# muellan/metacache

Measured on AMD Instinct MI355X. Metric: Mreads/min (150 bp), higher is better.
Workload: dtype u32

## Files before the change

### metacache_amd/csrc/gw_kernels.hip

```cpp
#include "device_common.h"

#include <algorithm>
#include <cstdlib>

namespace mcamd {

namespace {

constexpr uint32_t kGwNone = 0xFFFFFFFFu;
constexpr uint32_t kGwRounds = 128;
constexpr uint32_t kGwLoads = kGwRounds / 16;

struct __attribute__((packed, aligned(4))) U4 { uint32_t x, y, z, w; };

__device__ __forceinline__ uint32_t gw_block_shift(uint32_t maxWin)
{
    const uint32_t D = maxWin > 1 ? maxWin - 1 : 1;
    const uint32_t A = 32u - (uint32_t)__builtin_clz(64u * D - 1u);
    return A < 8u ? 8u : A;
}

template <uint32_t T1LOG2, uint32_t T2LOG2>
struct GwBloom {
    static constexpr uint32_t kW1 = (1u << T1LOG2) / 32, kW2 = (1u << T2LOG2) / 32, kWords = kW1 + kW2;
// ... 572 lines not shown
__device__ __forceinline__ uint32_t gw_count_numbers(const uint32_t (&v)[PER], uint2* slots, uint32_t* ck, const uint32_t lane)
{
    constexpr uint32_t kByteMask = ((1u << LOG2S) - 1u) << 3;
    char* base = reinterpret_cast<char*>(slots);
    auto key_at = [&](uint32_t off) -> uint32_t* { return reinterpret_cast<uint32_t*>(base + off); };
    uint32_t off[PER], old[PER];
    bool coll = false;
#pragma unroll
    for (uint32_t r = 0; r < PER; ++r) {
        off[r] = gw_slot<LOG2S>(v[r]);
        old[r] = v[r] != kGwNone ? atomicCAS(key_at(off[r]), kGwNone, v[r]) : v[r];
        coll = coll || (old[r] != kGwNone && old[r] != v[r]);
    }
    if (__ballot(coll)) {
#pragma unroll
        for (uint32_t r = 0; r < PER; ++r) {
            if (old[r] != kGwNone && old[r] != v[r]) {
                uint32_t o = off[r];
                for (;;) {
                    o = (o + 8u) & kByteMask;
                    old[r] = atomicCAS(key_at(o), kGwNone, v[r]);
                    if (old[r] == kGwNone || old[r] == v[r]) break;
                }
                off[r] = o;
            }
        }
    }
    uint32_t C = 0;
#pragma unroll
    for (uint32_t r = 0; r < PER; ++r) {
        if (v[r] != kGwNone) atomicAdd(key_at(off[r]) + 1, 1u);
        const bool claimed = v[r] != kGwNone && old[r] == kGwNone;
        const uint64_t m = __ballot(claimed);
        if (claimed) {
            const uint32_t at = __builtin_amdgcn_mbcnt_hi((uint32_t)(m >> 32), __builtin_amdgcn_mbcnt_lo((uint32_t)m, C));
            if (CKCAP == 0xFFFFFFFFu || at < CKCAP) ck[at] = off[r];
        }
        C += (uint32_t)__popcll(m);
    }
    return C;
}

template <uint32_t LOG2S, uint32_t PER, bool TAX>
__device__ __forceinline__ uint32_t gw_pick(const uint32_t* ck, const uint32_t C, uint2* slots, const uint32_t lane, const uint32_t maxWin,
                                            const uint32_t K, const uint32_t* __restrict__ taxkey, const DeviceTable& tab,
                                            uint32_t& owv, uint32_t& owh, uint32_t& owd)
{
    constexpr uint32_t kByteMask = ((1u << LOG2S) - 1u) << 3;
    const char* base = reinterpret_cast<const char*>(slots);
    uint32_t v[PER], R[PER];
#pragma unroll
    for (uint32_t r = 0; r < PER; ++r) {
        const uint2 c = r * 64 + lane < C ? *reinterpret_cast<const uint2*>(base + ck[r * 64 + lane]) : make_uint2(kGwNone, 0u);
        v[r] = c.x; R[r] = c.y;
    }
    uint32_t tgt[TAX ? PER : 1], thi[TAX ? PER : 1];
    if constexpr (TAX) {
#pragma unroll
        for (uint32_t r = 0; r < PER; ++r) tgt[r] = v[r] != kGwNone ? tab.gwDir[v[r] >> tab.gwDirShift] : 0u;
    }
    for (uint32_t d = 1; d < maxWin; ++d) {
        uint2 kc[PER]; uint32_t o[PER];
        bool chain = false;
#pragma unroll
        for (uint32_t r = 0; r < PER; ++r) {
            o[r] = gw_slot<LOG2S>(v[r] - d);
            kc[r] = *reinterpret_cast<const uint2*>(base + o[r]);
            if (v[r] == kGwNone) kc[r].x = kGwNone;
            chain = chain || (kc[r].x != v[r] - d && kc[r].x != kGwNone);
        }
        if (__ballot(chain)) {
#pragma unroll
            for (uint32_t r = 0; r < PER; ++r)
                while (kc[r].x != v[r] - d && kc[r].x != kGwNone) { o[r] = (o[r] + 8u) & kByteMask; kc[r] = *reinterpret_cast<const uint2*>(base + o[r]); }
        }
#pragma unroll
        for (uint32_t r = 0; r < PER; ++r)
            if (kc[r].x == v[r] - d) R[r] = ((R[r] & 0xFFFFu) + kc[r].y) | (d << 16);
    }
    uint32_t ptax[TAX ? PER : 1];
    if constexpr (TAX) {
#pragma unroll
        for (uint32_t r = 0; r < PER; ++r) {
            thi[r] = v[r] != kGwNone ? tab.gwBase[tgt[r] + 1] : 0u;
            while (v[r] != kGwNone && v[r] >= thi[r]) { ++tgt[r]; thi[r] = tab.gwBase[tgt[r] + 1]; }
            ptax[r] = v[r] != kGwNone ? taxkey[tgt[r]] : 0u;
        }
    }
    uint32_t live = 0;
#pragma unroll
    for (uint32_t r = 0; r < PER; ++r) {
        bool ok = v[r] != kGwNone;
        if constexpr (TAX) ok = ok && ptax[r] != 0;
        live |= ok ? (1u << r) : 0u;
    }
    uint32_t strong = 0;
    uint32_t wv = kGwNone, wh = 0, wd = 0;
    for (uint32_t rnd = 0; rnd < K; ++rnd) {
        uint32_t hh = 0, hv = kGwNone, hd = 0, hg = 0;
#pragma unroll
        for (uint32_t r = 0; r < PER; ++r) {
            const uint32_t h = R[r] & 0xFFFFu;
            const bool take = ((live >> r) & 1u) && (h > hh || (h == hh && v[r] < hv));
            if (take) { hh = h; hv = v[r]; hd = R[r] >> 16; if constexpr (TAX) hg = ptax[r]; }
        }
        const uint32_t mh = wave_max_u32(hh);
        if (mh == 0) break;
        const uint32_t mv = wave_min_u32(hh == mh ? hv : kGwNone);
        const uint32_t winner = __ffsll((unsigned long long)__ballot(hh == mh && hv == mv)) - 1;
        const uint32_t d = rdlane(hd, winner);
        if constexpr (TAX) {
            const uint32_t g = rdlane(hg, winner);
#pragma unroll
            for (uint32_t r = 0; r < PER; ++r) if (ptax[r] == g) live &= ~(1u << r);
        } else {
            const uint32_t from = mv - tab.gwGap, span = 2u * tab.gwGap;
#pragma unroll
            for (uint32_t r = 0; r < PER; ++r) if (v[r] - from <= span) live &= ~(1u << r);
        }
        if (lane == rnd) { wv = mv; wh = mh; wd = d; }
        strong += mh >= 2 ? 1u : 0u;
    }
    owv = wv; owh = wh; owd = wd;
    return strong;
}

template <bool TAX>
__device__ __forceinline__ bool gw_winners_out(const uint32_t lane, const uint32_t K, const uint32_t wv, const uint32_t wh, const uint32_t wd,
                                               const uint32_t wt, const uint32_t wlo, const uint32_t whi, mc_candidate_dev* __restrict__ out,
                                               uint32_t (&pickLo)[kLaneK], uint32_t (&pickHi)[kLaneK])
{
    bool again = false;
    if constexpr (!TAX) {
#pragma unroll
        for (uint32_t i = 0; i + 1 < kLaneK; ++i) {
            const uint32_t ti = rdlane(wt, i);
            again = again || (__ballot(lane > i && lane < K && wt == ti && ti != 0xFFFFFFFFu) != 0);
        }
    }
#pragma unroll
    for (uint32_t i = 0; i < kLaneK; ++i) { pickLo[i] = rdlane(wlo, i); pickHi[i] = rdlane(whi, i); }
    if (lane < K) {
        mc_candidate_dev e; e.tgt = wt; e.hits = wh; e.end = wv - wlo; e.beg = e.end - wd;
        if (wv == kGwNone) { e.tgt = 0xFFFFFFFFu; e.hits = 0; e.beg = 0; e.end = 0; }
        out[lane] = e;
    }
    return again;
}

}

namespace {

struct GwPend {
    bool pend = false;
    uint32_t q = 0, wv = kGwNone, wh = 0, wd = 0, dir = 0, b0 = 0, b1 = 0, b2 = 0;
    __device__ __forceinline__ void bases(const DeviceTable& tab)
    {
        if (pend && wv != kGwNone) { b0 = tab.gwBase[dir]; b1 = tab.gwBase[dir + 1]; b2 = tab.gwBase[min(dir + 2, tab.gwTargets)]; }
    }
    template <bool TAX>
    __device__ __forceinline__ void finish(const uint32_t lane, const uint32_t K, const DeviceTable& tab, const Workspace& ws, mc_candidate_dev* __restrict__ cands)
    {
        if (!pend) return;
        uint32_t t = 0xFFFFFFFFu, lo = 0, hi = 0;
        if (wv != kGwNone) {
            t = dir; lo = b0; hi = b1;
            if (wv >= b1) { ++t; lo = b1; hi = b2; }
            while (wv >= hi) { ++t; lo = hi; hi = tab.gwBase[t + 1]; }
        }
        uint32_t plo[kLaneK], phi[kLaneK];
        const bool again = gw_winners_out<TAX>(lane, K, wv, wh, wd, t, lo, hi, cands + (size_t)q * K, plo, phi);
        if (lane == 0) {
            if (again) { ws.hitScan[q] = ws.qstat[q].hits; ws.qflag[q] = kFlagCands; }
            else ws.qflag[q] = kFlagDone;
        }
        pend = false;
    }
};

template <uint32_t LOG2S, bool TAX, bool DEFER, bool LONG = false, class GetV, class EntF>
__device__ __forceinline__ bool gw_count_read(const uint32_t q, EntF&& entf, const uint32_t n2, const uint32_t maxWin, GetV&& getv,
                                              uint2* slots, uint32_t* ck, uint64_t* T, const uint32_t lane, const uint32_t grp, const uint32_t sub4,
                                              const uint32_t K, const uint32_t* __restrict__ taxkey, const DeviceTable& tab, const Workspace& ws,
                                              mc_candidate_dev* __restrict__ cands, GwPend& P)
{
    constexpr uint32_t kSlots = 1u << LOG2S, kList = kSlots / 2;
    {
        uint4* k4 = reinterpret_cast<uint4*>(slots);
#pragma unroll
        for (uint32_t i = 0; i < kSlots * 8 / 16 / 64; ++i) k4[i * 64 + lane] = make_uint4(kGwNone, 0u, kGwNone, 0u);
    }
    wave_lds_sync();
    uint32_t pickLo[kLaneK], pickHi[kLaneK];
#pragma unroll
    for (uint32_t i = 0; i < kLaneK; ++i) { pickLo[i] = 0; pickHi[i] = 0; }
    uint32_t strong = 0, wv = kGwNone, wh = 0, wd = 0;
    bool again = false;
    mc_candidate_dev* out = cands + (size_t)q * K;
    if constexpr (DEFER) P.bases(tab);
    uint32_t C = 0;
    auto body = [&](auto perc) {
        constexpr uint32_t PER = decltype(perc)::value;
        uint32_t v[PER];
#pragma unroll
        for (uint32_t r = 0; r < PER; ++r) v[r] = getv(r);
        C = gw_count_numbers<LOG2S, PER, LONG ? kList : 0xFFFFFFFFu>(v, slots, ck, lane);
    };
    const uint32_t per = (n2 + 63u) / 64u;
    if constexpr (LOG2S == 9) {
        if (per <= 1) body(std::integral_constant<uint32_t, 1>{});
        else if (per <= 2) body(std::integral_constant<uint32_t, 2>{});
        else if (per <= 3) body(std::integral_constant<uint32_t, 3>{});
        else if (!LONG || per <= 4) body(std::integral_constant<uint32_t, 4>{});
        else if constexpr (LONG) {
            if (per <= 6) body(std::integral_constant<uint32_t, 6>{});
            else body(std::integral_constant<uint32_t, 8>{});
        }
    } else if constexpr (LOG2S == 10) {
        if (per <= 6) body(std::integral_constant<uint32_t, 6>{});
        else body(std::integral_constant<uint32_t, 8>{});
    } else {
        if (per <= 10) body(std::integral_constant<uint32_t, 10>{});
        else if (per <= 12) body(std::integral_constant<uint32_t, 12>{});
        else body(std::integral_constant<uint32_t, kList / 64>{});
    }
    C = __builtin_amdgcn_readfirstlane(C);
    wave_lds_sync();
    if constexpr (LONG) {
        if (C > kList) {
            if constexpr (DEFER) P.template finish<TAX>(lane, K, tab, ws, cands);
            wave_lds_sync();
            return false;
        }
    }
    auto pick = [&](auto perc) {
        constexpr uint32_t PER = decltype(perc)::value;
        strong = gw_pick<LOG2S, PER, TAX>(ck, C, slots, lane, maxWin, K, taxkey, tab, wv, wh, wd);
    };
    if (C <= 64) pick(std::integral_constant<uint32_t, 1>{});
    else if (C <= 128) pick(std::integral_constant<uint32_t, 2>{});
    else if (C <= 256) pick(std::integral_constant<uint32_t, 4>{});
    else if constexpr (LOG2S >= 10) {
        if (C <= 512) pick(std::integral_constant<uint32_t, 8>{});
        else if constexpr (LOG2S >= 11) pick(std::integral_constant<uint32_t, 16>{});
    }
    strong = __builtin_amdgcn_readfirstlane(strong);
    if constexpr (DEFER) {
        P.template finish<TAX>(lane, K, tab, ws, cands);
        if (strong >= K) {
            P.pend = true; P.q = q; P.wv = wv; P.wh = wh; P.wd = wd;
            P.dir = wv != kGwNone ? tab.gwDir[wv >> tab.gwDirShift] : 0u;
            wave_lds_sync();
            return true;
        }
    }
    {
        uint32_t wt = 0xFFFFFFFFu, wlo = 0, whi = 0;
        if (wv != kGwNone) tab.gw_target_bounds(wv, wt, wlo, whi);
        again = gw_winners_out<TAX>(lane, K, wv, wh, wd, wt, wlo, whi, out, pickLo, pickHi);
    }
    bool done = true;
    if (again) {
        if (lane == 0) { ws.hitScan[q] = ws.qstat[q].hits; ws.qflag[q] = kFlagCands; }
        done = false;
    } else if (strong < K) {
        const uint2 r6 = entf();
        const uint32_t fbase = r6.x, nent = r6.y;
        if (TAX || nent > kBigEnt) {
            if (lane == 0) { ws.hitScan[q] = ws.qstat[q].hits; ws.qflag[q] = kFlagCands; }
            done = false;
        } else if constexpr (!TAX) {
            wave_lds_sync();
            const uint32_t sz = lane < nent ? (ws.psize[fbase + lane] & 0xFFFFu) : 0u;
            const uint64_t pay = lane < nent ? ws.ppay[fbase + lane] : 0ull;
            const uint32_t myR = sz > 1 ? (sz + 15u) >> 4 : 0u;
            const uint32_t incl = wave_incl_scan_u32(myR, lane), Rc = rdlane(incl, 63), start = incl - myR;
            uint32_t best[kLaneK];
#pragma unroll
            for (uint32_t i = 0; i < kLaneK; ++i) best[i] = kGwNone;
            uint32_t seen = 0;
            auto visit = [&](uint32_t g, bool valid) {
                if (!valid) return;
                bool skip = false;
#pragma unroll
                for (uint32_t i = 0; i < kLaneK; ++i) skip = skip || (i < strong && g - pickLo[i] < pickHi[i] - pickLo[i]);
                if (skip) return;
                ++seen;
                uint32_t c = g;
#pragma unroll
                for (uint32_t i = 0; i < kLaneK; ++i) { const uint32_t lo = min(best[i], c); c = max(best[i], c); best[i] = lo; }
            };
            visit(sz == 1 ? tab.gw_of(pay) : kGwNone, sz == 1);
            for (uint32_t r0 = 0; r0 < Rc; r0 += kGwRounds) {
                for (uint32_t i = lane; i < kGwRounds; i += 64) if (r0 + i >= Rc) T[i] = 0ull;
                const uint32_t jlo = r0 > start ? r0 - start : 0u, jhi = min(myR, r0 + kGwRounds > start ? r0 + kGwRounds - start : 0u);
                for (uint32_t j = jlo; j < jhi; ++j) T[start + j - r0] = (pay + 16ull * j) | ((uint64_t)min(16u, sz - 16u * j) << 40);
                wave_lds_sync();
#pragma unroll
                for (uint32_t u = 0; u < kGwLoads; ++u) {
                    const uint64_t rd = T[u * 16 + grp];
                    const int32_t rem = (int32_t)(uint32_t)(rd >> 40) - (int32_t)sub4;
                    if (rem > 0) {
                        const U4 t = *reinterpret_cast<const U4*>(tab.values32 + (rd & 0xFFFFFFFFFFull) + sub4);
                        visit(t.x, true); visit(t.y, rem > 1); visit(t.z, rem > 2); visit(t.w, rem > 3);
                    }
                }
                wave_lds_sync();
            }
            const bool dropped = seen > kLaneK;
            bool unsure = false;
            for (uint32_t rnd = strong; rnd < K; ++rnd) {
                if (__ballot(dropped && best[0] == kGwNone)) { unsure = true; break; }
                const uint32_t m = wave_min_u32(best[0]);
                mc_candidate_dev e; e.tgt = 0xFFFFFFFFu; e.hits = 0; e.beg = 0; e.end = 0;
                if (m != kGwNone) {
                    const uint32_t t = tab.gw_target(m), lo = tab.gwBase[t], hi = tab.gwBase[t + 1];
                    e.tgt = t; e.hits = 1; e.beg = e.end = m - lo;
                    uint32_t kept[kLaneK];
#pragma unroll
                    for (uint32_t i = 0; i < kLaneK; ++i) kept[i] = kGwNone;
                    uint32_t n = 0;
#pragma unroll
                    for (uint32_t i = 0; i < kLaneK; ++i) {
                        const bool stay = best[i] != kGwNone && !(best[i] - lo < hi - lo);
#pragma unroll
                        for (uint32_t j = 0; j < kLaneK; ++j) if (stay && j == n) kept[j] = best[i];
                        n += stay ? 1u : 0u;
                    }
#pragma unroll
                    for (uint32_t i = 0; i < kLaneK; ++i) best[i] = kept[i];
                }
                if (lane == 0) out[rnd] = e;
            }
            if (unsure) {
                if (lane == 0) { ws.hitScan[q] = ws.qstat[q].hits; ws.qflag[q] = kFlagCands; }
                done = false;
            }
        }
    }
    if (done && lane == 0) ws.qflag[q] = kFlagDone;
    wave_lds_sync();
    return true;
}

}

#ifndef MC_GW_COUNT_WPE
#define MC_GW_COUNT_WPE 6
#endif
template <uint32_t LOG2S, uint32_t WAVES, bool TAX>
__global__ __launch_bounds__(WAVES * 64, LOG2S == 9 ? MC_GW_COUNT_WPE : LOG2S == 10 ? 5 : 1) void gw_count_kernel(BatchView b, uint32_t s, DeviceTable tab, Workspace ws, uint32_t K,
                                                                                             const uint32_t* __restrict__ taxkey, mc_candidate_dev* __restrict__ cands,
                                                                                             uint32_t minN2)
{
    constexpr uint32_t kSlots = 1u << LOG2S, kList = kSlots / 2;
    static_assert(kGwRounds * 8 <= kSlots * 8, "step D's round table lives in the slot table, which is done with by then");
    __shared__ __attribute__((aligned(16))) uint2 slotS[WAVES][kSlots];
    __shared__ uint32_t ckS[WAVES][kList];
    const uint32_t lane = threadIdx.x & 63u, wave = __builtin_amdgcn_readfirstlane(threadIdx.x >> 6);
    uint2* slots = slotS[wave];
    uint32_t* ck = ckS[wave];
    uint64_t* T = reinterpret_cast<uint64_t*>(slotS[wave]);
    const uint32_t total = ws.midCount[kCntFilter];
    const uint4* __restrict__ work = ws.midList + list_at(kListFiltered, b.n);
    const uint4* __restrict__ work6 = ws.midList + list_at(kListFilter, b.n);
    const uint32_t nWaves = gridDim.x * WAVES;
    const uint32_t w0 = blockIdx.x * WAVES + wave;
    const uint32_t grp = lane >> 2, sub4 = (lane & 3u) * 4u;
    const uint32_t* __restrict__ pool = reinterpret_cast<const uint32_t*>(ws.bigPool);
    constexpr uint32_t kPre = LOG2S <= 10 ? kList / 64 : 1;
    uint32_t pre[kPre];
    auto fetch = [&](uint32_t off, uint32_t n) {
        if constexpr (LOG2S <= 10) {
#pragma unroll
            for (uint32_t r = 0; r < kPre; ++r) pre[r] = r * 64 + lane < n ? pool[off + r * 64 + lane] : kGwNone;
        }
    };
    constexpr bool kDefer = LOG2S <= 10;
    GwPend P;
    const uint32_t nmine = LOG2S == 9 ? total : ws.midCount[LOG2S == 10 ? kCnt512 : kCnt1024];
    const uint32_t kStep = LOG2S == 9 ? 64u : min(8u, max(1u, (nmine + nWaves - 1) / nWaves));
    const uint32_t* __restrict__ side = ws.sideList + list_at(LOG2S == 10 ? kSide512 : kSide1024, b.n);
    for (uint32_t chunk = w0 * kStep; chunk < nmine; chunk += nWaves * kStep) {
      const bool inb = lane < kStep && chunk + lane < nmine;
      const uint32_t myW = LOG2S == 9 ? chunk + lane : (inb ? side[chunk + lane] : 0u);
      const uint4 myRec = inb ? work[myW] : make_uint4(0, 0, kGwFallback, 0);
      uint64_t todo = __ballot(myRec.z <= kList && (minN2 == 0 || myRec.z > minN2) && myRec.w <= kHashWin);
      if (todo) { const uint32_t j = (uint32_t)__ffsll((unsigned long long)todo) - 1; fetch(rdlane(myRec.y, j), rdlane(myRec.z, j)); }
      while (todo) {
        const uint32_t j = (uint32_t)__ffsll((unsigned long long)todo) - 1;
        todo &= todo - 1;
        const uint32_t w = rdlane(myW, j), q = rdlane(myRec.x, j), n2 = rdlane(myRec.z, j), maxWin = rdlane(myRec.w, j);
        const uint32_t* __restrict__ src = pool + rdlane(myRec.y, j);
        uint32_t cur[kPre];
#pragma unroll
        for (uint32_t r = 0; r < kPre; ++r) cur[r] = pre[r];
        if (todo) { const uint32_t jn = (uint32_t)__ffsll((unsigned long long)todo) - 1; fetch(rdlane(myRec.y, jn), rdlane(myRec.z, jn)); }
        gw_count_read<LOG2S, TAX, kDefer>(q, [&]() -> uint2 { const uint4 r6 = work6[w]; return make_uint2(r6.y, r6.z & 0xFFFu); }, n2, maxWin, [&](uint32_t r) -> uint32_t {
            if constexpr (LOG2S <= 10) return cur[r < kPre ? r : 0];
            else return r * 64 + lane < n2 ? src[r * 64 + lane] : kGwNone;
        }, slots, ck, T, lane, grp, sub4, K, taxkey, tab, ws, cands, P);
      }
    }
    if constexpr (kDefer) { P.bases(tab); P.template finish<TAX>(lane, K, tab, ws, cands); }
}

constexpr uint32_t kGwCounted = 0x80000000u;

template <uint32_t WAVES, uint32_t TLOG2, bool TAX, uint32_t WPE = MC_GW_FILTER_WPE, bool LOOKUP = false>
__global__ __launch_bounds__(WAVES * 64, WPE) void gw_filter_count_kernel(BatchView b, DeviceTable tab, Workspace ws, uint32_t K, const uint32_t* __restrict__ taxkey,
                                                                                 mc_candidate_dev* __restrict__ cands, const uint32_t s)
{
    using Bloom = GwBloom<TLOG2, TLOG2>;
    constexpr uint32_t kKeep = WPE >= 6 ? 384 : 512;
    static_assert(kGwRounds * 8 >= 256 * 4, "the distinct numbers' slots take the place of the round table");
    constexpr bool kSeven = WPE >= 7;
    __shared__ __attribute__((aligned(16))) uint32_t bitS[WAVES][Bloom::kWords];
    __shared__ __attribute__((aligned(16))) uint64_t roundS[kSeven ? 1 : WAVES][kSeven ? 1 : kGwRounds];
    __shared__ __attribute__((aligned(16))) uint32_t keptS[WAVES][kKeep];
    const uint32_t lane = threadIdx.x & 63u, wave = __builtin_amdgcn_readfirstlane(threadIdx.x >> 6);
    uint32_t* bits = bitS[wave];
    uint64_t* T = kSeven ? reinterpret_cast<uint64_t*>(bits) : roundS[kSeven ? 0 : wave];
    uint32_t* kept = keptS[wave];
    const uint32_t total = LOOKUP ? b.n : ws.midCount[kCntFilter];
    uint4* const work = ws.midList + list_at(kListFilter, b.n);
    uint4* __restrict__ outRec = ws.midList + list_at(kListFiltered, b.n);
    const uint32_t nWaves = gridDim.x * WAVES;
    const uint32_t w0 = blockIdx.x * WAVES + wave;
    auto load_rec = [&](uint32_t w) -> uint4 { return (!LOOKUP && w < total) ? work[w] : make_uint4(0, 0, 0, 0); };
    const uint64_t sliceCap = ws.bigPoolCap / nWaves;
    uint32_t* const slice = reinterpret_cast<uint32_t*>(ws.bigPool) + (uint64_t)w0 * sliceCap;
    uint64_t sliceUsed = (LOOKUP && ws.sliceFill) ? ws.sliceFill[w0] : 0u;
    uint32_t deferred = 0;
    uint4 rec = load_rec(w0), recNext = load_rec(w0 + nWaves);
    uint32_t esz = 0; uint64_t epay = 0;
    auto load_entries = [&](const uint4& r) {
        if constexpr (LOOKUP) return;
        const uint32_t ne = (r.z >> 12) <= kGwSmallH ? min(r.z & 0xFFFu, 64u) : 0u;
        esz = lane < ne ? ws.psize[r.y + lane] : 0u;
        epay = lane < ne ? ws.ppay[r.y + lane] : 0ull;
    };
    load_entries(rec);
    constexpr uint32_t kLkSkip = 0xFFFFFFFFu;
    auto load_meta = [&](uint32_t q) -> uint2 {
        if (!LOOKUP || q >= b.n) return make_uint2(kLkSkip, 0u);
        const uint32_t o0 = ws.winOff[q], nf = (ws.winOff[q + 1] - o0) * s;
        return (ws.qflag[q] == kFlagProbe && nf <= 64u) ? make_uint2(o0 * s, nf) : make_uint2(kLkSkip, 0u);
    };
    auto load_feat = [&](const uint2& m) -> uint32_t { return (m.x != kLkSkip && lane < m.y) ? ws.features[m.x + lane] : 0xFFFFFFFFu; };
    uint2 m0 = load_meta(w0), m1 = load_meta(w0 + nWaves), m2 = load_meta(w0 + 2 * nWaves);
    uint32_t lkFeat = 0xFFFFFFFFu, lkNfeat = 0; uint64_t lkEnt = 0;
    if constexpr (LOOKUP) {
        const uint32_t f0 = load_feat(m0);
        lkFeat = load_feat(m1);
        lkNfeat = (uint32_t)__popcll(__ballot(f0 != 0xFFFFFFFFu));
        lkEnt = f0 != 0xFFFFFFFFu ? tab.direct[f0] : 0ull;
    }
    const uint32_t grp = lane >> 2, sub4 = (lane & 3u) * 4u;
    GwPend P;
    for (uint32_t w = w0; w < total; w += nWaves) {
        uint32_t q, nent, H, maxWin, sz, fbase = 0; uint64_t pay;
        uint32_t rix = 0xFFFFFFFFu;
        if constexpr (!LOOKUP) {
            q = rec.x; nent = rec.z & 0xFFFu; H = rec.z >> 12; maxWin = rec.w;
            sz = esz & 0xFFFFu; pay = epay;
            rec = recNext;
            recNext = load_rec(w + 2 * nWaves);
            load_entries(rec);
        } else {
            const uint2 cur = m0; const uint64_t e = lkEnt; const uint32_t nfeat = lkNfeat;
            lkNfeat = (uint32_t)__popcll(__ballot(lkFeat != 0xFFFFFFFFu));
            lkEnt = lkFeat != 0xFFFFFFFFu ? tab.direct[lkFeat] : 0ull;
            lkFeat = load_feat(m2);
            m0 = m1; m1 = m2; m2 = load_meta(w + 3 * nWaves);
            if (cur.x == kLkSkip) continue;
            q = w; fbase = cur.x;
            sz = (uint32_t)e & 0xFFFFu; pay = direct_payload(e);
            const uint64_t fm = __ballot(sz != 0u), sm = __ballot(sz == 1u);
            nent = (uint32_t)__popcll(fm);
            const uint32_t n1 = (uint32_t)__popcll(sm), lsz = sz > 1u ? sz : 0u;
            const uint32_t lincl = wave_incl_scan_u32(lsz, lane);
            H = n1 + rdlane(lincl, 63);
            maxWin = b.maxWin ? b.maxWin[q] : b.maxWinUniform;
            if (lane == 0) { QueryStat qs; qs.hits = H; qs.nfeat = nfeat; qs.nfound = nent; qs.nsteps = nfeat; ws.qstat[q] = qs; }
            if (H == 0) {
                if (lane < K) { mc_candidate_dev ev; ev.tgt = 0xFFFFFFFFu; ev.hits = 0; ev.beg = 0; ev.end = 0; cands[(size_t)q * K + lane] = ev; }
                if (lane == 0) { ws.hitScan[q] = 0u; ws.qflag[q] = kFlagDone; }
                continue;
            }
            {
                const uint32_t below = __builtin_amdgcn_mbcnt_hi((uint32_t)(fm >> 32), __builtin_amdgcn_mbcnt_lo((uint32_t)fm, 0u));
                const uint32_t sbelow = __builtin_amdgcn_mbcnt_hi((uint32_t)(sm >> 32), __builtin_amdgcn_mbcnt_lo((uint32_t)sm, 0u));
                if (sz != 0u) {
                    const uint32_t slot = sz == 1u ? sbelow : n1 + (below - sbelow);
                    const uint32_t off = sz == 1u ? slot : n1 + lincl - lsz;
                    ws.psize[fbase + slot] = sz | ((off & 0xFFFu) << 16);
                    ws.ppay[fbase + slot] = pay;
                } else if (lane < cur.y) ws.psize[fbase + nent + (lane - below)] = 0u;
            }
            const bool hashOK = nent <= kHashEnt && maxWin <= kHashWin;
            const bool bigOK = H > ws.bigMin && H > 64u && nent <= 0xFFFu && maxWin <= tab.gwGap && H <= kMaxHitsPerQuery;
            const uint32_t cls = bigOK ? kClassFilter : H <= 64 ? kListMid64 : H <= 128 ? (hashOK ? kListHash256 : kListMid128) : H <= kMidMax ? (hashOK ? kListHash256 : kListMid256)
                               : (H <= kHashMax && hashOK) ? (H <= kHashMax / 2 ? kListHash512 : kListHash1024) : kClassWave;
            if (lane == 0) {
                ws.hitScan[q] = (H <= kMaxHitsPerQuery && H > kLdsCap && !(cls >= kListHash512 && cls != kClassWave)) ? H : 0u;
                ws.qflag[q] = cls != kClassWave ? kFlagMid : kFlagCands;
                if (cls != kClassWave && cls != kClassFilter) {
                    const uint32_t at = atomicAdd(&ws.midCount[class_counter(cls)], 1u);
                    ws.midList[list_at(class_list(cls), b.n) + at] = make_uint4(q, fbase, nent | (H << 12), maxWin);
                }
            }
            if (cls != kClassFilter) continue;
        }
        auto slot_of = [&]() -> uint32_t {
            if constexpr (!LOOKUP) return w;
            else {
                if (rix == 0xFFFFFFFFu) {
                    uint32_t at = 0;
                    if (lane == 0) { at = atomicAdd(&ws.midCount[kCntFilter], 1u); work[at] = make_uint4(q, fbase, nent | (H << 12), maxWin); }
                    rix = rdlane(at, 0);
                }
                return rix;
            }
        };
        const uint32_t myR = sz > 1 ? (sz + 15u) >> 4 : 0u;
        const uint32_t incl = wave_incl_scan_u32(myR, lane), Rc = rdlane(incl, 63);
        if (H > kGwSmallH || nent > 64u || Rc > kGwRounds || maxWin > tab.gwGap || sliceCap - sliceUsed < kGwRounds * 16u + 64u) {
            const uint32_t at = slot_of();
            if (lane == 0) outRec[at] = make_uint4(q, 0u, kGwDefer, maxWin);
            ++deferred;
            continue;
        }
        auto clear_bits = [&]() {
            uint4* z4 = reinterpret_cast<uint4*>(bits);
#pragma unroll
            for (uint32_t i = 0; i < Bloom::kWords / 4 / 64; ++i) z4[i * 64 + lane] = make_uint4(0, 0, 0, 0);
        };
        if constexpr (!kSeven) clear_bits();
        gw_fill_rounds_scan(T, kept, lane, Rc, incl - myR, myR, sz, pay);
        wave_lds_sync();
        const GwFrame F(maxWin);
        const uint32_t nl = (Rc + 15u) >> 4;
        uint4 x[kGwLoads];
        gw_load_rounds(T, tab.values32, grp, sub4, x, nl);
        uint32_t rems = 0;
        if constexpr (kSeven) {
            rems = gw_pack_rems(T, grp, sub4, nl);
            wave_lds_sync();
            clear_bits();
            wave_lds_sync();
        }
        auto take_rounds = [&](auto check, GwSink& S) {
            constexpr bool CHECK = decltype(check)::value;
            if constexpr (kSeven) gw_take_rounds_packed<Bloom, CHECK>(bits, rems, F, S, x, nl);
            else gw_take_rounds<Bloom, CHECK>(bits, T, F, S, grp, sub4, x, nl);
        };
        const uint32_t sv = sz == 1 ? tab.gw_of(pay) : kGwNone;
        if (sv != kGwNone) Bloom::mark(bits, sv >> F.A);
        gw_mark_rounds<Bloom>(bits, x, F.A, nl);
        wave_lds_sync();
        const bool here = maxWin <= kHashWin;
        uint32_t n2;
        if (here) {
            GwSink S{kept, kKeep, 0u};
            gw_take<Bloom>(bits, F, S, sv, sv != kGwNone);
            take_rounds(std::true_type{}, S);
            n2 = S.n2;
        } else {
            GwSink S{slice + sliceUsed, (uint32_t)min((uint64_t)kGwMaxKept, sliceCap - sliceUsed), 0u};
            gw_take<Bloom>(bits, F, S, sv, sv != kGwNone);
            take_rounds(std::false_type{}, S);
            n2 = S.n2;
        }
        if (here && n2 <= kKeep) {
            if constexpr (!LOOKUP) { if (lane == 0) outRec[w] = make_uint4(q, 0u, kGwCounted | n2, maxWin); }
            wave_lds_sync();
            const bool counted = gw_count_read<9, TAX, true, true>(q, [&]() -> uint2 {
                                            if constexpr (LOOKUP) { wave_mem_sync(); return make_uint2(fbase, nent); }
                                            else { const uint4 r6 = work[w]; return make_uint2(r6.y, r6.z & 0xFFFu); }
                                        }, n2, maxWin,
                                        [&](uint32_t r) -> uint32_t { return r * 64 + lane < n2 ? kept[r * 64 + lane] : kGwNone; },
                                        reinterpret_cast<uint2*>(bits), kSeven ? kept : reinterpret_cast<uint32_t*>(T), kSeven ? reinterpret_cast<uint64_t*>(kept) : T,
                                        lane, grp, sub4, K, taxkey, tab, ws, cands, P);
            if (!counted && kSeven) {
                const uint32_t at = slot_of();
                if (lane == 0) outRec[at] = make_uint4(q, 0u, kGwDefer, maxWin);
                ++deferred;
                wave_lds_sync();
            } else if (!counted) {
#pragma unroll
                for (uint32_t r = 0; r < kKeep / 64; ++r) if (r * 64 + lane < n2) slice[sliceUsed + r * 64 + lane] = kept[r * 64 + lane];
                const uint32_t at = slot_of();
                if (lane == 0) outRec[at] = make_uint4(q, (uint32_t)((uint64_t)w0 * sliceCap + sliceUsed), n2, maxWin);
                sliceUsed += n2;
                wave_lds_sync();
            }
            continue;
        }
        if (here) {
            GwSink S{slice + sliceUsed, (uint32_t)min((uint64_t)kGwMaxKept, sliceCap - sliceUsed), 0u};
            gw_take<Bloom>(bits, F, S, sv, sv != kGwNone);
            take_rounds(std::false_type{}, S);
            n2 = S.n2;
        }
        const uint32_t room = (uint32_t)min((uint64_t)kGwMaxKept, sliceCap - sliceUsed);
        const bool fallback = n2 > room;
        const uint32_t at = slot_of();
        if (lane == 0) {
            if (fallback) { ws.hitScan[q] = H; ws.qflag[q] = kFlagCands; outRec[at] = make_uint4(q, 0u, kGwFallback, maxWin); }
            else outRec[at] = make_uint4(q, (uint32_t)((uint64_t)w0 * sliceCap + sliceUsed), n2, maxWin);
        }
        if (!fallback) sliceUsed += n2;
        wave_lds_sync();
    }
    P.bases(tab); P.template finish<TAX>(lane, K, tab, ws, cands);
    if (lane == 0) {
        if (ws.sliceFill) ws.sliceFill[w0] = (uint32_t)sliceUsed;
        if (deferred) atomicAdd(&ws.midCount[kCntSecond], deferred);
    }
}

constexpr uint32_t kGwBigSorted = 8192;

template <bool TAX>
__device__ __forceinline__ void gw_sorted_scan(const uint32_t* __restrict__ g, const uint32_t first, const uint32_t end, const uint32_t D,
                                               const DeviceTable& tab, const uint32_t* __restrict__ taxkey, const uint32_t K, uint32_t* ring,
                                               const uint32_t lane, LaneCand (&top)[kLaneK], uint32_t (&toptax)[kLaneK])
{
    uint32_t cT = 0xFFFFFFFFu, cHits = 0, cBeg = 0, cEnd = 0, cLo = 0, cHi = 0;
    uint32_t lowFst = 0;
    uint32_t gnext = first + lane < end ? g[first + lane] : 0xFFFFFFFFu;
    uint32_t dnext = gnext != 0xFFFFFFFFu ? tab.gwDir[gnext >> tab.gwDirShift] : 0u;
    for (uint32_t base = first; base < end; base += 64) {
        const uint32_t cnt = min(64u, end - base), ei = base + lane;
        const bool valid = lane < cnt;
        const uint32_t gi = gnext, di = dnext;
        gnext = ei + 64u < end ? g[ei + 64u] : 0xFFFFFFFFu;
        ring[ei & 127u] = gi;
        wave_lds_sync();
        const uint32_t want = gi - D;
        const uint32_t rlo = base >= first + 64u ? base - 64u : first;
        uint32_t lo = 0, hi = 0;
        bool glob = false;
        if (valid) {
            if (lowFst >= rlo) { lo = lowFst; hi = ei; }
            else if (ring[rlo & 127u] < want) { lo = rlo + 1u; hi = ei; }
            else { lo = lowFst; hi = rlo; glob = true; }
        }
        while (__ballot(!glob && lo < hi)) {
            const uint32_t mid = (lo + hi) >> 1;
            if (!glob && lo < hi) { if (ring[mid & 127u] < want) lo = mid + 1u; else hi = mid; }
        }
        while (__ballot(glob && lo < hi)) {
            const uint32_t mid = (lo + hi) >> 1;
            if (glob && lo < hi) { if (g[mid] < want) lo = mid + 1u; else hi = mid; }
        }
        const uint32_t fst = lo;
        const uint32_t gf = !valid ? 0u : fst >= rlo ? ring[fst & 127u] : g[fst];
        lowFst = rdlane(fst, cnt - 1u);
        uint32_t t = 0xFFFFFFFFu, tlo = 0, thi = 0;
        const bool inCur = cT != 0xFFFFFFFFu && (gi - cLo) < (cHi - cLo);
        if (valid) {
            if (inCur) { t = cT; tlo = cLo; thi = cHi; }
            else {
                t = di;
                const uint32_t b0 = tab.gwBase[t], b1 = tab.gwBase[t + 1], b2 = tab.gwBase[min(t + 2, tab.gwTargets)];
                tlo = b0; thi = b1;
                if (gi >= b1) { ++t; tlo = b1; thi = b2; }
                while (gi >= thi) { ++t; tlo = thi; thi = tab.gwBase[t + 1]; }
            }
        }
        if (cT != 0xFFFFFFFFu && rdlane(t, 0) != cT && lane == 0) {
            LaneCand c; c.tgt = cT; c.hits = cHits; c.beg = cBeg; c.end = cEnd;
            top_insert(top, toptax, c, K, TAX ? taxkey : nullptr, 0xFFFFFFFFu);
        }
        uint32_t val = valid ? (((ei - fst + 1u) << 6) | (63u - lane)) : 0u;
#pragma unroll
        for (uint32_t d = 1; d < 64; d <<= 1) {
            const uint32_t ov = (uint32_t)__shfl_up((int)val, d), ot = (uint32_t)__shfl_up((int)t, d);
            if (lane >= d && ot == t) val = max(val, ov);
        }
        const uint32_t tnext = (uint32_t)__shfl_down((int)t, 1);
        const bool tail = valid && (lane + 1u >= cnt || tnext != t);
        const uint32_t wl = 63u - (val & 63u);
        LaneCand c; c.tgt = t; c.hits = val >> 6;
        c.beg = (uint32_t)__shfl((int)gf, (int)wl) - tlo; c.end = (uint32_t)__shfl((int)gi, (int)wl) - tlo;
        if (t == cT && cHits >= c.hits) { c.hits = cHits; c.beg = cBeg; c.end = cEnd; }
        const bool last = base + 64u >= end;
        if (tail && (last || lane + 1u < cnt)) top_insert(top, toptax, c, K, TAX ? taxkey : nullptr, 0xFFFFFFFFu);
        cT = rdlane(c.tgt, cnt - 1u); cHits = rdlane(c.hits, cnt - 1u); cBeg = rdlane(c.beg, cnt - 1u); cEnd = rdlane(c.end, cnt - 1u);
        cLo = rdlane(tlo, cnt - 1u); cHi = rdlane(thi, cnt - 1u);
        dnext = gnext != 0xFFFFFFFFu ? tab.gwDir[gnext >> tab.gwDirShift] : 0u;
    }
    wave_lds_sync();
}

template <bool TAX, class Put>
__device__ __forceinline__ uint32_t gw_sorted_rounds(LaneCand (&top)[kLaneK], uint32_t (&toptax)[kLaneK], const uint32_t K, Put&& put)
{
    uint32_t strong = 0;
    for (uint32_t rnd = 0; rnd < K; ++rnd) {
        const uint32_t mh = wave_max_u32(top[0].hits);
        mc_candidate_dev ev; ev.tgt = 0xFFFFFFFFu; ev.hits = 0; ev.beg = 0; ev.end = 0;
        uint32_t mtax = 0;
        if (mh != 0) {
            const uint32_t mt = wave_min_u32(top[0].hits == mh ? top[0].tgt : 0xFFFFFFFFu);
            const uint32_t me = wave_min_u32(top[0].hits == mh && top[0].tgt == mt ? top[0].end : 0xFFFFFFFFu);
            const uint32_t winner = __ffsll((unsigned long long)__ballot(top[0].hits == mh && top[0].tgt == mt && top[0].end == me)) - 1;
            ev.tgt = mt; ev.hits = mh; ev.end = me; ev.beg = rdlane(top[0].beg, winner);
            mtax = rdlane(toptax[0], winner);
            strong += mh >= 2 ? 1u : 0u;
            LaneCand kept[kLaneK]; uint32_t ktax[kLaneK];
#pragma unroll
            for (uint32_t i = 0; i < kLaneK; ++i) { kept[i].tgt = 0xFFFFFFFFu; kept[i].hits = 0; kept[i].beg = 0; kept[i].end = 0; ktax[i] = 0; }
            uint32_t nk = 0;
#pragma unroll
            for (uint32_t i = 0; i < kLaneK; ++i) {
                const bool stay = top[i].hits != 0 && (TAX ? toptax[i] != mtax : top[i].tgt != mt);
#pragma unroll
                for (uint32_t jj = 0; jj < kLaneK; ++jj) if (stay && jj == nk) { kept[jj] = top[i]; ktax[jj] = toptax[i]; }
                nk += stay ? 1u : 0u;
            }
#pragma unroll
            for (uint32_t i = 0; i < kLaneK; ++i) { top[i] = kept[i]; toptax[i] = ktax[i]; }
        }
        put(rnd, ev, mtax);
    }
    return strong;
}

constexpr uint32_t kGwFewBig = 1024;
template <bool TAX, bool BIG>
__global__ __launch_bounds__(BIG ? 1024 : 256) void gw_sorted_cands_kernel(BatchView b, DeviceTable tab, Workspace ws, uint32_t K, const uint32_t* __restrict__ taxkey,
                                                                           mc_candidate_dev* __restrict__ cands)
{
    constexpr uint32_t kWaves = BIG ? 16u : 4u;
    __shared__ uint32_t ringS[kWaves][128];
    __shared__ mc_candidate_dev pickS[kWaves][kLaneK];
    __shared__ uint32_t ptaxS[kWaves][kLaneK];
    const uint32_t lane = threadIdx.x & 63u, wave = __builtin_amdgcn_readfirstlane(threadIdx.x >> 6);
    uint32_t* ring = ringS[wave];
    const uint4* __restrict__ work = ws.midList + list_at(kListFiltered, b.n);
    const uint32_t* __restrict__ side = ws.sideList + list_at(kSideSorted, b.n);
    auto finish = [&](uint32_t q, uint32_t strong) {
        if (lane == 0) {
            if (strong < K) { ws.hitScan[q] = ws.qstat[q].hits; ws.qflag[q] = kFlagCands; }
            else ws.qflag[q] = kFlagDone;
        }
    };
    if constexpr (!BIG) {
        const uint32_t nWaves = gridDim.x * 4, w0 = blockIdx.x * 4 + wave;
        const uint32_t nmine = ws.midCount[kCntSorted];
        uint32_t lo = 0, hi = nmine;
        while (lo < hi) { const uint32_t mid = (lo + hi) >> 1; if (work[side[mid]].z > kGwBigSorted) lo = mid + 1u; else hi = mid; }
        const uint32_t nbig = min(lo, kGwFewBig);
        if (w0 == 0 && lane == 0) ws.midCount[kCntSortedBig] = nbig;
        for (uint32_t i = nbig + w0; i < nmine; i += nWaves) {
            const uint32_t w = side[i];
            const uint4 rec = work[w];
            const uint32_t q = rec.x, n = rec.z, maxWin = rec.w;
            LaneCand top[kLaneK];
            uint32_t toptax[kLaneK];
#pragma unroll
            for (uint32_t j = 0; j < kLaneK; ++j) { top[j].tgt = 0xFFFFFFFFu; top[j].hits = 0; top[j].beg = 0; top[j].end = 0; toptax[j] = 0; }
            gw_sorted_scan<TAX>(ws.bigPool2 + rec.y, 0u, n, maxWin - 1u, tab, taxkey, K, ring, lane, top, toptax);
            mc_candidate_dev* out = cands + (size_t)q * K;
            const uint32_t strong = gw_sorted_rounds<TAX>(top, toptax, K, [&](uint32_t rnd, const mc_candidate_dev& ev, uint32_t) { if (lane == 0) out[rnd] = ev; });
            finish(q, strong);
// ... 109 lines not shown
```

Measured before the change: 20410.

## Defer writing per-query entry arrays until a fallback path needs them

In the lookup path, per-feature psize/ppay entries are no longer written for every query up front. They are written only when a query is classified away from the filter path, deferred, or falls back to the candidate pipeline. Queries finished in-kernel instead re-read features and the direct table on demand, or skip the stores entirely. This cuts global stores and a scan for the common case, at the cost of recomputing lookups when a restore is needed and more complex control flow.

```diff
diff --git a/metacache_amd/csrc/gw_kernels.hip b/metacache_amd/csrc/gw_kernels.hip
--- a/metacache_amd/csrc/gw_kernels.hip
+++ b/metacache_amd/csrc/gw_kernels.hip
@@ -748,6 +748,59 @@
 
 namespace {
 
+__device__ __forceinline__ void gw_store_entries(const uint32_t fbase, const uint32_t nf, const uint32_t sz, const uint64_t pay, const Workspace& ws,
+                                                 const uint32_t lane)
+{
+    const uint64_t fm = __ballot(sz != 0u), sm = __ballot(sz == 1u);
+    const uint32_t nent = (uint32_t)__popcll(fm), n1 = (uint32_t)__popcll(sm), lsz = sz > 1u ? sz : 0u;
+    const uint32_t lincl = wave_incl_scan_u32(lsz, lane);
+    const uint32_t below = __builtin_amdgcn_mbcnt_hi((uint32_t)(fm >> 32), __builtin_amdgcn_mbcnt_lo((uint32_t)fm, 0u));
+    const uint32_t sbelow = __builtin_amdgcn_mbcnt_hi((uint32_t)(sm >> 32), __builtin_amdgcn_mbcnt_lo((uint32_t)sm, 0u));
+    if (sz != 0u) {
+        const uint32_t slot = sz == 1u ? sbelow : n1 + (below - sbelow);
+        const uint32_t off = sz == 1u ? slot : n1 + lincl - lsz;
+        ws.psize[fbase + slot] = sz | ((off & 0xFFFu) << 16);
+        ws.ppay[fbase + slot] = pay;
+    } else if (lane < nf) ws.psize[fbase + nent + (lane - below)] = 0u;
+}
+
+struct GwEnt { uint32_t nent, sz; uint64_t pay; };
+struct GwEntStored {
+    const uint4* rec; const Workspace& ws; uint32_t lane;
+    __device__ __forceinline__ GwEnt entries() const
+    {
+        const uint4 r6 = *rec;
+        const uint32_t fbase = r6.y, nent = r6.z & 0xFFFu;
+        const bool mine = nent <= kBigEnt && lane < nent;
+        return GwEnt{nent, mine ? (ws.psize[fbase + lane] & 0xFFFFu) : 0u, mine ? ws.ppay[fbase + lane] : 0ull};
+    }
+    __device__ __forceinline__ uint2 restore(uint32_t) const { return make_uint2(0u, 0u); }
+};
+struct GwEntLookup {
+    uint32_t q, s; const DeviceTable& tab; const Workspace& ws; uint32_t lane;
+    __device__ __forceinline__ void load(const uint32_t r, uint32_t& fbase, uint32_t& nf, uint32_t& sz, uint64_t& pay) const
+    {
+        const uint32_t o0 = ws.winOff[r];
+        fbase = o0 * s; nf = min((ws.winOff[r + 1] - o0) * s, 64u);
+        const uint32_t f = lane < nf ? ws.features[fbase + lane] : 0xFFFFFFFFu;
+        const uint64_t e = f != 0xFFFFFFFFu ? tab.direct[f] : 0ull;
+        sz = (uint32_t)e & 0xFFFFu; pay = direct_payload(e);
+    }
+    __device__ __forceinline__ GwEnt entries() const
+    {
+        uint32_t fbase, nf, sz; uint64_t pay;
+        load(q, fbase, nf, sz, pay);
+        return GwEnt{(uint32_t)__popcll(__ballot(sz != 0u)), sz, pay};
+    }
+    __device__ __forceinline__ uint2 restore(const uint32_t r) const
+    {
+        uint32_t fbase, nf, sz; uint64_t pay;
+        load(r, fbase, nf, sz, pay);
+        gw_store_entries(fbase, nf, sz, pay, ws, lane);
+        return make_uint2(fbase, (uint32_t)__popcll(__ballot(sz != 0u)) | (wave_sum_u32(sz) << 12));
+    }
+};
+
 struct GwPend {
     bool pend = false;
     uint32_t q = 0, wv = kGwNone, wh = 0, wd = 0, dir = 0, b0 = 0, b1 = 0, b2 = 0;
@@ -755,8 +808,9 @@
     {
         if (pend && wv != kGwNone) { b0 = tab.gwBase[dir]; b1 = tab.gwBase[dir + 1]; b2 = tab.gwBase[min(dir + 2, tab.gwTargets)]; }
     }
-    template <bool TAX>
-    __device__ __forceinline__ void finish(const uint32_t lane, const uint32_t K, const DeviceTable& tab, const Workspace& ws, mc_candidate_dev* __restrict__ cands)
+    template <bool TAX, class Ent>
+    __device__ __forceinline__ void finish(const uint32_t lane, const uint32_t K, const DeviceTable& tab, const Workspace& ws, mc_candidate_dev* __restrict__ cands,
+                                           const Ent& ent)
     {
         if (!pend) return;
         uint32_t t = 0xFFFFFFFFu, lo = 0, hi = 0;
@@ -771,12 +825,13 @@
             if (again) { ws.hitScan[q] = ws.qstat[q].hits; ws.qflag[q] = kFlagCands; }
             else ws.qflag[q] = kFlagDone;
         }
+        if (again) ent.restore(q);
         pend = false;
     }
 };
 
-template <uint32_t LOG2S, bool TAX, bool DEFER, bool LONG = false, class GetV, class EntF>
-__device__ __forceinline__ bool gw_count_read(const uint32_t q, EntF&& entf, const uint32_t n2, const uint32_t maxWin, GetV&& getv,
+template <uint32_t LOG2S, bool TAX, bool DEFER, bool LONG = false, class GetV, class Ent>
+__device__ __forceinline__ bool gw_count_read(const uint32_t q, const Ent& ent, const uint32_t n2, const uint32_t maxWin, GetV&& getv,
                                               uint2* slots, uint32_t* ck, uint64_t* T, const uint32_t lane, const uint32_t grp, const uint32_t sub4,
                                               const uint32_t K, const uint32_t* __restrict__ taxkey, const DeviceTable& tab, const Workspace& ws,
                                               mc_candidate_dev* __restrict__ cands, GwPend& P)
@@ -825,7 +880,7 @@
     wave_lds_sync();
     if constexpr (LONG) {
         if (C > kList) {
-            if constexpr (DEFER) P.template finish<TAX>(lane, K, tab, ws, cands);
+            if constexpr (DEFER) P.template finish<TAX>(lane, K, tab, ws, cands, ent);
             wave_lds_sync();
             return false;
         }
@@ -843,7 +898,7 @@
     }
     strong = __builtin_amdgcn_readfirstlane(strong);
     if constexpr (DEFER) {
-        P.template finish<TAX>(lane, K, tab, ws, cands);
+        P.template finish<TAX>(lane, K, tab, ws, cands, ent);
         if (strong >= K) {
             P.pend = true; P.q = q; P.wv = wv; P.wh = wh; P.wd = wd;
             P.dir = wv != kGwNone ? tab.gwDir[wv >> tab.gwDirShift] : 0u;
@@ -857,19 +912,15 @@
         again = gw_winners_out<TAX>(lane, K, wv, wh, wd, wt, wlo, whi, out, pickLo, pickHi);
     }
     bool done = true;
-    if (again) {
-        if (lane == 0) { ws.hitScan[q] = ws.qstat[q].hits; ws.qflag[q] = kFlagCands; }
-        done = false;
-    } else if (strong < K) {
-        const uint2 r6 = entf();
-        const uint32_t fbase = r6.x, nent = r6.y;
-        if (TAX || nent > kBigEnt) {
-            if (lane == 0) { ws.hitScan[q] = ws.qstat[q].hits; ws.qflag[q] = kFlagCands; }
+    if (again) done = false;
+    else if (strong < K) {
+        const GwEnt e1 = ent.entries();
+        if (TAX || e1.nent > kBigEnt) {
             done = false;
         } else if constexpr (!TAX) {
             wave_lds_sync();
-            const uint32_t sz = lane < nent ? (ws.psize[fbase + lane] & 0xFFFFu) : 0u;
-            const uint64_t pay = lane < nent ? ws.ppay[fbase + lane] : 0ull;
+            const uint32_t sz = e1.sz;
+            const uint64_t pay = e1.pay;
             const uint32_t myR = sz > 1 ? (sz + 15u) >> 4 : 0u;
             const uint32_t incl = wave_incl_scan_u32(myR, lane), Rc = rdlane(incl, 63), start = incl - myR;
             uint32_t best[kLaneK];
@@ -929,13 +980,14 @@
                 }
                 if (lane == 0) out[rnd] = e;
             }
-            if (unsure) {
-                if (lane == 0) { ws.hitScan[q] = ws.qstat[q].hits; ws.qflag[q] = kFlagCands; }
-                done = false;
-            }
-        }
-    }
-    if (done && lane == 0) ws.qflag[q] = kFlagDone;
+            if (unsure) done = false;
+        }
+    }
+    if (lane == 0) {
+        if (done) ws.qflag[q] = kFlagDone;
+        else { ws.hitScan[q] = ws.qstat[q].hits; ws.qflag[q] = kFlagCands; }
+    }
+    if (!done) ent.restore(q);
     wave_lds_sync();
     return true;
 }
@@ -993,13 +1045,13 @@
 #pragma unroll
         for (uint32_t r = 0; r < kPre; ++r) cur[r] = pre[r];
         if (todo) { const uint32_t jn = (uint32_t)__ffsll((unsigned long long)todo) - 1; fetch(rdlane(myRec.y, jn), rdlane(myRec.z, jn)); }
-        gw_count_read<LOG2S, TAX, kDefer>(q, [&]() -> uint2 { const uint4 r6 = work6[w]; return make_uint2(r6.y, r6.z & 0xFFFu); }, n2, maxWin, [&](uint32_t r) -> uint32_t {
+        gw_count_read<LOG2S, TAX, kDefer>(q, GwEntStored{work6 + w, ws, lane}, n2, maxWin, [&](uint32_t r) -> uint32_t {
             if constexpr (LOG2S <= 10) return cur[r < kPre ? r : 0];
             else return r * 64 + lane < n2 ? src[r * 64 + lane] : kGwNone;
         }, slots, ck, T, lane, grp, sub4, K, taxkey, tab, ws, cands, P);
       }
     }
-    if constexpr (kDefer) { P.bases(tab); P.template finish<TAX>(lane, K, tab, ws, cands); }
+    if constexpr (kDefer) { P.bases(tab); P.template finish<TAX>(lane, K, tab, ws, cands, GwEntStored{work6, ws, lane}); }
 }
 
 constexpr uint32_t kGwCounted = 0x80000000u;
@@ -1056,7 +1108,7 @@
     const uint32_t grp = lane >> 2, sub4 = (lane & 3u) * 4u;
     GwPend P;
     for (uint32_t w = w0; w < total; w += nWaves) {
-        uint32_t q, nent, H, maxWin, sz, fbase = 0; uint64_t pay;
+        uint32_t q, nent, H, maxWin, sz, fbase = 0, nslot = 0; uint64_t pay;
         uint32_t rix = 0xFFFFFFFFu;
         if constexpr (!LOOKUP) {
             q = rec.x; nent = rec.z & 0xFFFu; H = rec.z >> 12; maxWin = rec.w;
@@ -1071,29 +1123,16 @@
             lkFeat = load_feat(m2);
             m0 = m1; m1 = m2; m2 = load_meta(w + 3 * nWaves);
             if (cur.x == kLkSkip) continue;
-            q = w; fbase = cur.x;
+            q = w; fbase = cur.x; nslot = cur.y;
             sz = (uint32_t)e & 0xFFFFu; pay = direct_payload(e);
-            const uint64_t fm = __ballot(sz != 0u), sm = __ballot(sz == 1u);
-            nent = (uint32_t)__popcll(fm);
-            const uint32_t n1 = (uint32_t)__popcll(sm), lsz = sz > 1u ? sz : 0u;
-            const uint32_t lincl = wave_incl_scan_u32(lsz, lane);
-            H = n1 + rdlane(lincl, 63);
+            nent = (uint32_t)__popcll(__ballot(sz != 0u));
+            H = wave_sum_u32(sz);
             maxWin = b.maxWin ? b.maxWin[q] : b.maxWinUniform;
             if (lane == 0) { QueryStat qs; qs.hits = H; qs.nfeat = nfeat; qs.nfound = nent; qs.nsteps = nfeat; ws.qstat[q] = qs; }
             if (H == 0) {
                 if (lane < K) { mc_candidate_dev ev; ev.tgt = 0xFFFFFFFFu; ev.hits = 0; ev.beg = 0; ev.end = 0; cands[(size_t)q * K + lane] = ev; }
                 if (lane == 0) { ws.hitScan[q] = 0u; ws.qflag[q] = kFlagDone; }
                 continue;
-            }
-            {
-                const uint32_t below = __builtin_amdgcn_mbcnt_hi((uint32_t)(fm >> 32), __builtin_amdgcn_mbcnt_lo((uint32_t)fm, 0u));
-                const uint32_t sbelow = __builtin_amdgcn_mbcnt_hi((uint32_t)(sm >> 32), __builtin_amdgcn_mbcnt_lo((uint32_t)sm, 0u));
-                if (sz != 0u) {
-                    const uint32_t slot = sz == 1u ? sbelow : n1 + (below - sbelow);
-                    const uint32_t off = sz == 1u ? slot : n1 + lincl - lsz;
-                    ws.psize[fbase + slot] = sz | ((off & 0xFFFu) << 16);
-                    ws.ppay[fbase + slot] = pay;
-                } else if (lane < cur.y) ws.psize[fbase + nent + (lane - below)] = 0u;
             }
             const bool hashOK = nent <= kHashEnt && maxWin <= kHashWin;
             const bool bigOK = H > ws.bigMin && H > 64u && nent <= 0xFFFu && maxWin <= tab.gwGap && H <= kMaxHitsPerQuery;
@@ -1107,14 +1146,18 @@
                     ws.midList[list_at(class_list(cls), b.n) + at] = make_uint4(q, fbase, nent | (H << 12), maxWin);
                 }
             }
-            if (cls != kClassFilter) continue;
-        }
-        auto slot_of = [&]() -> uint32_t {
+            if (cls != kClassFilter) { gw_store_entries(fbase, nslot, sz, pay, ws, lane); continue; }
+        }
+        const GwEntLookup lkEntries{q, s, tab, ws, lane};
+        uint32_t lateH = 0;
+        auto slot_of = [&](const bool late = true) -> uint32_t {
             if constexpr (!LOOKUP) return w;
             else {
                 if (rix == 0xFFFFFFFFu) {
+                    const uint2 r6 = late ? lkEntries.restore(q) : make_uint2(fbase, nent | (H << 12));
+                    lateH = r6.y >> 12;
                     uint32_t at = 0;
-                    if (lane == 0) { at = atomicAdd(&ws.midCount[kCntFilter], 1u); work[at] = make_uint4(q, fbase, nent | (H << 12), maxWin); }
+                    if (lane == 0) { at = atomicAdd(&ws.midCount[kCntFilter], 1u); work[at] = make_uint4(q, r6.x, r6.y, maxWin); }
                     rix = rdlane(at, 0);
                 }
                 return rix;
@@ -1123,7 +1166,8 @@
         const uint32_t myR = sz > 1 ? (sz + 15u) >> 4 : 0u;
         const uint32_t incl = wave_incl_scan_u32(myR, lane), Rc = rdlane(incl, 63);
         if (H > kGwSmallH || nent > 64u || Rc > kGwRounds || maxWin > tab.gwGap || sliceCap - sliceUsed < kGwRounds * 16u + 64u) {
-            const uint32_t at = slot_of();
+            if constexpr (LOOKUP) gw_store_entries(fbase, nslot, sz, pay, ws, lane);
+            const uint32_t at = slot_of(false);
             if (lane == 0) outRec[at] = make_uint4(q, 0u, kGwDefer, maxWin);
             ++deferred;
             continue;
@@ -1172,13 +1216,15 @@
         if (here && n2 <= kKeep) {
             if constexpr (!LOOKUP) { if (lane == 0) outRec[w] = make_uint4(q, 0u, kGwCounted | n2, maxWin); }
             wave_lds_sync();
-            const bool counted = gw_count_read<9, TAX, true, true>(q, [&]() -> uint2 {
-                                            if constexpr (LOOKUP) { wave_mem_sync(); return make_uint2(fbase, nent); }
-                                            else { const uint4 r6 = work[w]; return make_uint2(r6.y, r6.z & 0xFFFu); }
-                                        }, n2, maxWin,
+            auto count = [&](const auto& ent) {
+                return gw_count_read<9, TAX, true, true>(q, ent, n2, maxWin,
                                         [&](uint32_t r) -> uint32_t { return r * 64 + lane < n2 ? kept[r * 64 + lane] : kGwNone; },
                                         reinterpret_cast<uint2*>(bits), kSeven ? kept : reinterpret_cast<uint32_t*>(T), kSeven ? reinterpret_cast<uint64_t*>(kept) : T,
                                         lane, grp, sub4, K, taxkey, tab, ws, cands, P);
+            };
+            bool counted;
+            if constexpr (LOOKUP) counted = count(lkEntries);
+            else counted = count(GwEntStored{work + w, ws, lane});
             if (!counted && kSeven) {
                 const uint32_t at = slot_of();
                 if (lane == 0) outRec[at] = make_uint4(q, 0u, kGwDefer, maxWin);
@@ -1204,13 +1250,15 @@
         const bool fallback = n2 > room;
         const uint32_t at = slot_of();
         if (lane == 0) {
-            if (fallback) { ws.hitScan[q] = H; ws.qflag[q] = kFlagCands; outRec[at] = make_uint4(q, 0u, kGwFallback, maxWin); }
+            if (fallback) { ws.hitScan[q] = LOOKUP ? lateH : H; ws.qflag[q] = kFlagCands; outRec[at] = make_uint4(q, 0u, kGwFallback, maxWin); }
             else outRec[at] = make_uint4(q, (uint32_t)((uint64_t)w0 * sliceCap + sliceUsed), n2, maxWin);
         }
         if (!fallback) sliceUsed += n2;
         wave_lds_sync();
     }
-    P.bases(tab); P.template finish<TAX>(lane, K, tab, ws, cands);
+    P.bases(tab);
+    if constexpr (LOOKUP) P.template finish<TAX>(lane, K, tab, ws, cands, GwEntLookup{0u, s, tab, ws, lane});
+    else P.template finish<TAX>(lane, K, tab, ws, cands, GwEntStored{work, ws, lane});
     if (lane == 0) {
         if (ws.sliceFill) ws.sliceFill[w0] = (uint32_t)sliceUsed;
         if (deferred) atomicAdd(&ws.midCount[kCntSecond], deferred);
```

After: 20490, median of 3. No clear change (+0.4%).
